# catid/siamese

Hardware: AMD Instinct MI355X
Metric: device-resident GB/s encode+decode, 1400B pkts @20% loss; % HBM peak (higher is better)
Workload: dtype u8

## Files before the change

siamese_amd/csrc/decoder.cpp:

```cpp
#include "decoder.h"

#include <algorithm>
#include <atomic>
#include <cstdio>
#include <cstdlib>
#include <cstring>
#include <x86intrin.h>

namespace sgpu {

namespace {

inline unsigned popcount_range(uint64_t bits, unsigned begin, unsigned end)
{
    if (begin >= end)
        return 0;
    uint64_t mask = (end >= 64 ? ~0ULL : ((1ULL << end) - 1)) & ~((1ULL << begin) - 1);
    return (unsigned)__builtin_popcountll(bits & mask);
}

inline unsigned first_clear(uint64_t bits, unsigned from)
{
    if (from >= 64)
        return 64;
    const uint64_t inv = ~bits & (~0ULL << from);
    return inv ? (unsigned)__builtin_ctzll(inv) : 64;
}

}

DecoderCore::DecoderCore(Engine* eng, bool hostMirror)
    : eng_(eng), prog_(eng, 1), mirror_(hostMirror)
{
    adopt_spare();
    if (!res_)
        res_ = std::make_shared<Resolver>();
    res_->mirror = mirror_;
}

struct DecoderCore::Spare
{
    std::vector<DecSubwindowPtr> subwindows;
    std::vector<SiameseOriginalPacket> recovered;
    std::vector<unsigned> recoveredColumns;
    std::vector<RowInfo> rows;
    std::vector<ColInfo> cols;
    std::vector<uint8_t> colLane, colCx, colCx2;
    std::vector<uint32_t> pickCol;
    std::vector<uint8_t> mat;
    std::vector<unsigned> pivots;
    std::shared_ptr<Resolver> res;
    std::vector<Fix> lastDecoded;
    std::vector<RecPacket*> scratchRec;
    std::vector<unsigned> scratchLen;
    std::vector<SolveRow> scratchRows;
    std::vector<uint8_t> scratchCoef;
    std::vector<unsigned> geEnd;
    std::vector<DevBuf> chainReleases;
    std::vector<unsigned> chainColumns;
    std::vector<uint32_t> geOut;
};

void DecoderCore::adopt_spare()
{
    Spare* s = CapStash<Spare>::take();
    if (!s)
        return;
    subwindows_.swap(s->subwindows);
    recovered_.swap(s->recovered);
    recoveredColumns_.swap(s->recoveredColumns);
    rows_.swap(s->rows);
    cols_.swap(s->cols);
    colLane_.swap(s->colLane);
    colCx_.swap(s->colCx);
    colCx2_.swap(s->colCx2);
    pickCol_.swap(s->pickCol);
    mat_.swap(s->mat);
    pivots_.swap(s->pivots);
    res_.swap(s->res);
    lastDecoded_.swap(s->lastDecoded);
    scratchRec_.swap(s->scratchRec);
    scratchLen_.swap(s->scratchLen);
    scratchRows_.swap(s->scratchRows);
    scratchCoef_.swap(s->scratchCoef);
    geEnd_.swap(s->geEnd);
    chainReleases_.swap(s->chainReleases);
    chainSums_.recoveredColumns.swap(s->chainColumns);
    geOut_.swap(s->geOut);
    CapStash<Spare>::put_shell(s);
}

void DecoderCore::donate_spare()
{
    Spare* s = CapStash<Spare>::shell();
    subwindows_.clear();
    recovered_.clear();
    recoveredColumns_.clear();
    rows_.clear();
    cols_.clear();
    colLane_.clear();
    colCx_.clear();
    colCx2_.clear();
    pickCol_.clear();
    pivots_.clear();
    if (res_ && res_.use_count() == 1) {
        for (PendingDecode& pd : res_->pend) {
            pd.fixes.clear();
            pd.words.clear();
            pd.targets.clear();
            pd.base = 0;
            pd.m = 0;
            pd.serial = 0;
            pd.live = false;
            pd.done = false;
            pd.held = false;
        }
        res_->doneCount.store(0, std::memory_order_relaxed);
        res_->orphan = false;
        res_->out = nullptr;
        res_->outCount = 0;
        res_->outSerial = 0;
        res_->geOut.clear();
        res_->geDone = false;
    } else if (res_) {
        std::lock_guard<std::mutex> g(res_->mu);
        res_->orphan = true;
        res_->out = nullptr;
        res_->outCount = 0;
        res_.reset();
    }
    lastDecoded_.clear();
    scratchRec_.clear();
    scratchLen_.clear();
    scratchRows_.clear();
    scratchCoef_.clear();
    geEnd_.clear();
    chainReleases_.clear();
    chainSums_.recoveredColumns.clear();
    geOut_.clear();
    subwindows_.swap(s->subwindows);
    recovered_.swap(s->recovered);
    recoveredColumns_.swap(s->recoveredColumns);
    rows_.swap(s->rows);
    cols_.swap(s->cols);
    colLane_.swap(s->colLane);
    colCx_.swap(s->colCx);
    colCx2_.swap(s->colCx2);
    pickCol_.swap(s->pickCol);
    mat_.swap(s->mat);
    pivots_.swap(s->pivots);
    res_.swap(s->res);
    lastDecoded_.swap(s->lastDecoded);
    scratchRec_.swap(s->scratchRec);
    scratchLen_.swap(s->scratchLen);
    scratchRows_.swap(s->scratchRows);
    scratchCoef_.swap(s->scratchCoef);
    geEnd_.swap(s->geEnd);
    chainReleases_.swap(s->chainReleases);
    chainSums_.recoveredColumns.swap(s->chainColumns);
    geOut_.swap(s->geOut);
    CapStash<Spare>::give(s);
}

DecoderCore::~DecoderCore()
{
    for (RecPacket* r = head_; r;) {
        RecPacket* n = r->next;
        free_packet(r);
        r = n;
    }
    for (auto& sw : subwindows_) {
        for (DecSlot& s : sw->slot) {
            if (!s.inSlab)
                eng_->release(s.buf);
            s.buf = DevBuf();
            s.inSlab = false;
            s.bytes = 0;
            s.column = 0;
            s.header = 0;
            s.pending = false;
            if (s.hostp)
                s.hostp->clear();
        }
        sw->got = 0;
        sw->gotCount = 0;
        eng_->slab_release(sw->slab);
        sw->slab = Slab();
        sw->clean = true;
    }
    for (auto& lane : lanes_)
        for (Sum& s : lane)
            eng_->release(s.d.buf);
    if (geState_ == 2)
        chain_sums_commit();
    donate_spare();
}


bool DecoderCore::mark_got(unsigned column)
{
    const unsigned element = column_to_element(column);
    if (element >= count_) {
        disabled_ = true;
        return false;
    }
    DecSubwindow* sw = subwindows_[element / kSubwindow].get();
    sw->gotCount++;
    sw->got |= 1ULL << (element % kSubwindow);
    return element == nextExpected_;
}

unsigned DecoderCore::range_lost(unsigned start, unsigned end)
{
    if (start >= end)
        return 0;
    unsigned lost = 0;
    unsigned sub = start / kSubwindow;
    const unsigned bitStart = start % kSubwindow;
    if (bitStart > 0) {
        unsigned bitEnd = bitStart + end - start;
        if (bitEnd > kSubwindow)
            bitEnd = kSubwindow;
        lost += (bitEnd - bitStart) - popcount_range(subwindows_[sub]->got, bitStart, bitEnd);
        ++sub;
    }
    const unsigned subEnd = end / kSubwindow;
    for (unsigned i = sub; i < subEnd; ++i)
        lost += kSubwindow - subwindows_[i]->gotCount;
    if (subEnd >= sub) {
        const unsigned lastBits = end - subEnd * kSubwindow;
        if (lastBits > 0)
            lost += lastBits - popcount_range(subwindows_[subEnd]->got, 0, lastBits);
    }
    return lost;
}

unsigned DecoderCore::find_next_lost(unsigned start)
{
    if (start >= count_)
        return count_;
    const unsigned subEnd = (count_ + kSubwindow - 1) / kSubwindow;
    unsigned sub = start / kSubwindow;
    unsigned bit = start % kSubwindow;
    while (sub < subEnd) {
        const DecSubwindow* sw = subwindows_[sub].get();
        if (sw->gotCount < kSubwindow) {
            bit = first_clear(sw->got, bit);
            if (bit < kSubwindow) {
                const unsigned e = sub * kSubwindow + bit;
                return e > count_ ? count_ : e;
            }
        }
        bit = 0;
        ++sub;
    }
    return count_;
}

void DecoderCore::iterate_next_expected(unsigned start)
{
    if (nextExpected_ >= count_)
        return;
    nextExpected_ = find_next_lost(start);
}

bool DecoderCore::grow_window(unsigned end)
{
    const unsigned needed = (end + kLanes + kSubwindow - 1) / kSubwindow;
    while (subwindows_.size() < needed) {
        subwindows_.emplace_back(ObjPool<DecSubwindow>::get());
        subwindows_.back()->clean = false;
    }
    if (end > count_)
        count_ = end;
    return true;
}

bool DecoderCore::place(unsigned element, unsigned need)
{
    DecSubwindow* sw = subwindows_[element / kSubwindow].get();
    DecSlot& s = sw->slot[element % kSubwindow];
    release_slot(s);
    bool failed = false;
    s.buf = eng_->slab_slot(sw->slab, element % kSubwindow, need, &failed);
    s.inSlab = (bool)s.buf;
    if (!s.buf && !failed)
        s.buf = eng_->alloc(need);
    return (bool)s.buf;
}

SiameseResult DecoderCore::accept_original(unsigned element, unsigned column, unsigned header, unsigned dataBytes)
{
    if (!place(element, header + dataBytes)) {
        disabled_ = true;
        return Siamese_Disabled;
    }
    DecSubwindow* sw = subwindows_[element / kSubwindow].get();
    const unsigned bit = element % kSubwindow;
    DecSlot& s = sw->slot[bit];
    s.header = header;
    s.bytes = header + dataBytes;
    s.column = column;
    s.pending = false;

    sw->gotCount++;
    sw->got |= 1ULL << bit;

    if (element == nextExpected_) {
        iterate_next_expected(element + 1);
        list_delete_before(nextExpected_);
    }
    if (element >= region_.elementStart && element < region_.nextCheckStart)
        region_reset();

    stats_[SiameseDecoderStats_OriginalCount]++;
    stats_[SiameseDecoderStats_OriginalBytes] += dataBytes;
    return Siamese_Success;
}

SiameseResult DecoderCore::add_original(const SiameseOriginalPacket& packet, uint64_t deviceSrc)
{
    settle();
    if (dead())
        return Siamese_Disabled;
    const unsigned element = column_to_element(packet.PacketNum);
    if (column_delta_negative(element)) {
        stats_[SiameseDecoderStats_DupedOriginalCount]++;
        return Siamese_DuplicateData;
    }
    grow_window(element + 1);
    DecSlot& s = slot(element);
    if (s.bytes > 0) {
        stats_[SiameseDecoderStats_DupedOriginalCount]++;
        return Siamese_DuplicateData;
    }

    uint8_t hdr[kMaxLengthPrefix];
    const unsigned h = write_length_prefix(packet.DataBytes, hdr);
    const SiameseResult r = accept_original(element, packet.PacketNum, h, packet.DataBytes);
    if (r != Siamese_Success)
        return r;
    if (deviceSrc)
        prog_.ingest_device(s.buf, deviceSrc, packet.DataBytes, hdr, h);
    else
        prog_.ingest_host(s.buf, packet.Data, packet.DataBytes, hdr, h);
    if (mirror_) {
        s.host().resize(h + packet.DataBytes);
        std::memcpy(s.host().data(), hdr, h);
        std::memcpy(s.host().data() + h, packet.Data, packet.DataBytes);
    }
    return Siamese_Success;
}

SiameseResult DecoderCore::add_original_range(unsigned firstNum, uint64_t src, uint32_t srcStride,
                                              const unsigned* lens, unsigned fixedBytes, unsigned count,
                                              SiameseResult* results, unsigned* added)
{
    *added = 0;
    settle();
    struct
    {
        uint64_t dst = 0, src = 0;
        uint32_t stride = 0, n = 0, bytes = 0, h = 0;
        uint8_t hdr[kMaxLengthPrefix] = {};
    } run;
    auto close_run = [&] {
        if (run.n)
            prog_.ingest_run(run.dst, run.stride, run.src, srcStride, run.n, run.bytes, run.hdr, run.h);
        run.n = 0;
    };
    SiameseResult res = Siamese_Success;
    for (unsigned k = 0; k < count; ++k) {
        const unsigned num = (firstNum + k) & SIAMESE_PACKET_NUM_MAX;
        const unsigned bytes = lens ? lens[k] : fixedBytes;
        SiameseResult r = Siamese_Success;
        const unsigned element = column_to_element(num);
        if (bytes == 0 || bytes > SIAMESE_MAX_PACKET_BYTES)
            r = Siamese_InvalidInput;
        else if (dead())
            r = Siamese_Disabled;
        else if (column_delta_negative(element))
            r = Siamese_DuplicateData;
        else {
            grow_window(element + 1);
            if (slot(element).bytes > 0)
                r = Siamese_DuplicateData;
        }
        if (r == Siamese_DuplicateData)
            stats_[SiameseDecoderStats_DupedOriginalCount]++;
        if (r == Siamese_Success) {
            uint8_t hdr[kMaxLengthPrefix];
            const unsigned h = write_length_prefix(bytes, hdr);
            r = accept_original(element, num, h, bytes);
            if (r == Siamese_Success) {
                const DecSlot& s = slot(element);
                const uint64_t from = src + (uint64_t)k * srcStride;
                if (run.n && run.bytes == bytes && run.n < kIngestRunMax && s.buf.cap == run.stride &&
                    s.buf.addr() == run.dst + (uint64_t)run.n * run.stride &&
                    from == run.src + (uint64_t)run.n * srcStride)
                    ++run.n;
                else {
                    close_run();
                    run.dst = s.buf.addr();
                    run.src = from;
                    run.stride = s.buf.cap;
                    run.n = 1;
                    run.bytes = bytes;
                    run.h = h;
                    std::memcpy(run.hdr, hdr, sizeof(hdr));
                }
            }
        }
        if (results)
            results[k] = r;
        ++*added;
        if (r != Siamese_Success && r != Siamese_DuplicateData) {
            res = r;
            break;
        }
    }
    close_run();
    return res;
}


bool DecoderCore::grow_sum(DevSum& s, unsigned bytes)
{
    if (bytes <= s.bytes)
        return true;
    if (bytes > s.buf.cap) {
        DevBuf nb = eng_->alloc(bytes);
        if (!nb) {
            disabled_ = true;
            return false;
        }
        if (s.devValid) {
            prog_.lc_begin(nb.addr(), s.devValid, 0);
            prog_.lc_term(s.buf.addr(), s.devValid, 1);
            prog_.lc_end();
        }
        release_sum_buf(s.buf);
        s.buf = nb;
    }
    s.bytes = bytes;
    return true;
}

void DecoderCore::cover(unsigned lo, unsigned hi)
{
    uint32_t from = hi;
    WinEntry* w = prog_.rows_window(lo, hi, &from);
    for (unsigned e = from; e < hi; ++e, ++w) {
        const DecSlot& o = slot(e);
        w->src = o.bytes ? o.buf.addr() : 0;
        w->len = o.bytes;
        w->column = o.bytes ? o.column : 0;
    }
}

void DecoderCore::materialize(unsigned lane, unsigned s)
{
    DevSum& d = sum(lane, s).d;
    if (d.devValid >= d.bytes)
        return;
    const unsigned at = sum(lane, s).elementEnd;
    const unsigned lo = std::min(at, windowLo_);
    cover(lo, lo);
    prog_.rows_update(lane * kSums + s, d.buf.addr(), d.bytes, d.devValid, s, at, at);
    d.devValid = d.bytes;
}

static uint8_t sum_coeff(unsigned sumIndex, unsigned column)
{
    if (sumIndex == 0)
        return 1;
    const uint8_t cx = column_value(column);
    return sumIndex == 2 ? gf_sqr(cx) : cx;
}

DevSum& DecoderCore::get_sum(unsigned lane, unsigned s, unsigned elementEnd)
{
    Sum& S = sum(lane, s);
    unsigned element = S.elementEnd;
    if (element >= elementEnd)
        return S.d;

    LaneScan& ls = laneScan_[lane];
    unsigned end = element;
    if (!(ls.from == element && ls.to == elementEnd && ls.epoch == scanEpoch_)) {
        unsigned most = 0, cnt = 0;
        for (; end < elementEnd; end += kLanes) {
            const unsigned b = slot(end).bytes;
            if (b > 0) {
                most = std::max(most, b);
                ++cnt;
            }
        }
        ls.from = element;
        ls.to = elementEnd;
        ls.end = end;
        ls.most = most;
        ls.got = cnt;
        ls.epoch = scanEpoch_;
    }
    end = ls.end;
    const unsigned got = ls.got;
    const unsigned newBytes = std::max(S.d.bytes, ls.most);
    if (got > 0) {
        if (!grow_sum(S.d, newBytes))
            return S.d;
        cover(std::min(element, windowLo_), end - kLanes + 1);
        prog_.rows_update(lane * kSums + s, S.d.buf.addr(), S.d.bytes, S.d.devValid, s, element, end);
        S.d.devValid = S.d.bytes;
    }
    S.elementEnd = end;
    return S.d;
}

bool DecoderCore::plug_sum_holes(unsigned elementStart)
{
    for (unsigned column : recoveredColumns_) {
        const unsigned element = column_to_element(column);
        if (element >= count_)
            continue;
        const unsigned lane = column % kLanes;
        const unsigned laneStart = next_lane_element(elementStart, lane);
        for (unsigned s = 0; s < kSums; ++s) {
            Sum& S = sum(lane, s);
            if (element < laneStart || element >= S.elementEnd)
                continue;
            const DecSlot& o = slot(element);
            if (o.bytes == 0)
                return false;
            if (!grow_sum(S.d, o.bytes))
                return false;
            prog_.lc_begin(S.d.buf.addr(), S.d.bytes, S.d.devValid);
            prog_.lc_term(o.buf.addr(), o.bytes, sum_coeff(s, column));
            prog_.lc_end();
            account_elim(o.bytes);
            S.d.devValid = S.d.bytes;
        }
    }
    recoveredColumns_.clear();
    return true;
}

void DecoderCore::reset_sums(unsigned elementStart)
{
    for (unsigned lane = 0; lane < kLanes; ++lane) {
        const unsigned laneStart = next_lane_element(elementStart, lane);
        for (unsigned s = 0; s < kSums; ++s) {
            Sum& S = sum(lane, s);
            S.elementStart = laneStart;
            S.elementEnd = laneStart;
            S.d.bytes = 0;
            S.d.devValid = 0;
        }
    }
    recoveredColumns_.clear();
}

bool DecoderCore::start_sums(unsigned elementStart, unsigned bufferBytes)
{
    for (unsigned lane = 0; lane < kLanes; ++lane) {
        const unsigned laneStart = next_lane_element(elementStart, lane);
        for (unsigned s = 0; s < kSums; ++s) {
            Sum& S = sum(lane, s);
            if (S.d.bytes == 0) {
                S.elementEnd = laneStart;
            } else if (S.elementStart != laneStart) {
                S.elementEnd = laneStart;
                S.d.bytes = 0;
                S.d.devValid = 0;
            }
            S.elementStart = laneStart;
            if (!grow_sum(S.d, bufferBytes))
                return false;
        }
    }
    if (!recoveredColumns_.empty() && !plug_sum_holes(elementStart))
        return false;
    return true;
}


void DecoderCore::remove_elements()
{
    if (nextExpected_ < kRemoveThreshold)
        return;

    unsigned firstKept = 0;
    unsigned targetStart = 0, targetCount = 0, initialBytes = 0;
    bool seenSum = false;

    const RecPacket* r = head_;
    if (!r) {
        const RowMeta m = lastMeta_;
        const unsigned end = column_to_element(m.columnStart + m.sumCount);
        if (column_delta_negative(end) || end < m.ldpcCount) {
            disabled_ = true;
            return;
        }
        firstKept = end - m.ldpcCount;
        targetStart = m.columnStart;
        targetCount = m.sumCount;
        initialBytes = lastBytes_;
        if (m.sumCount > kCauchyThreshold)
            seenSum = true;
    } else {
        firstKept = r->elementStart;
        initialBytes = r->bytes;
        for (;;) {
            const unsigned sc = r->meta.sumCount;
            const unsigned cs = r->meta.columnStart;
            if (sc > kCauchyThreshold) {
                if (!seenSum) {
                    targetStart = cs;
                    targetCount = sc;
                    seenSum = true;
                } else if (cs != targetStart || sc < targetCount) {
                    const unsigned firstSum = column_to_element(cs);
                    if (firstSum >= count_) {
                        disabled_ = true;
                        return;
                    }
                    if (firstKept > firstSum)
                        firstKept = firstSum;
                }
            }
            r = r->next;
            if (!r)
                break;
            if (firstKept > r->elementStart)
                firstKept = r->elementStart;
            if (initialBytes < r->bytes)
                initialBytes = r->bytes;
        }
    }

    if (firstKept < kRemoveThreshold)
        return;

    const unsigned keptSub = firstKept / kSubwindow;
    const unsigned removed = keptSub * kSubwindow;

    if (seenSum) {
        unsigned sumElementStart = column_to_element(targetStart);
        if (sumColumnStart_ != targetStart || sumColumnCount_ > targetCount) {
            if (sumElementStart >= count_) {
                disabled_ = true;
                return;
            }
            reset_sums(sumElementStart);
            sumColumnStart_ = targetStart;
            sumColumnCount_ = targetCount;
        } else {
            if (sumElementStart >= count_)
                sumElementStart = 0;
            if (!start_sums(sumElementStart, initialBytes)) {
                disabled_ = true;
                return;
            }
        }
        ++scanEpoch_;
        for (unsigned lane = 0; lane < kLanes; ++lane) {
            for (unsigned s = 0; s < kSums; ++s) {
                get_sum(lane, s, removed);
                Sum& S = sum(lane, s);
                if (S.elementStart >= removed)
                    S.elementStart -= removed;
                else
                    S.elementStart = lane;
                S.elementEnd -= removed;
            }
        }
    } else {
        sumColumnCount_ = 0;
    }

    prog_.rows_seal();
    for (unsigned i = 0; i < keptSub; ++i) {
        DecSubwindow* sw = subwindows_[i].get();
        for (DecSlot& d : sw->slot)
            if (d.inSlab) {
                d.buf = DevBuf();
                d.inSlab = false;
            }
        eng_->slab_release(sw->slab);
        sw->reset();
    }
    std::rotate(subwindows_.begin(), subwindows_.begin() + keptSub, subwindows_.end());

    count_ -= removed;
    columnStart_ = element_to_column(removed);
    nextExpected_ -= removed;

    for (RecPacket* p = head_; p; p = p->next) {
        p->elementEnd -= removed;
        p->elementStart -= removed;
    }
    if (region_.elementStart < removed || region_.nextCheckStart < removed)
        region_reset();
    else {
        region_.elementStart -= removed;
        region_.nextCheckStart -= removed;
    }
    prevNextCheckStart_ = prevNextCheckStart_ > removed ? prevNextCheckStart_ - removed : 0;
}


void DecSubwindowRecycle::operator()(DecSubwindow* w) const
{
    if (!w->clean) {
        w->got = 0;
        w->gotCount = 0;
        w->slab = Slab();
        for (DecSlot& s : w->slot) {
            s.buf = DevBuf();
            s.inSlab = false;
            s.bytes = 0;
            s.column = 0;
            s.header = 0;
            s.pending = false;
            if (s.hostp)
                s.hostp->clear();
        }
        w->clean = true;
    }
    ObjPool<DecSubwindow>::put(w);
}

void DecoderCore::free_packet(RecPacket* r)
{
    eng_->release(r->buf);
    *r = RecPacket();
    ObjPool<RecPacket>::put(r);
}

void DecoderCore::list_insert(RecPacket* r, bool outOfOrder)
{
    RecPacket* prev = tail_;
    RecPacket* next = nullptr;
    const unsigned rs = r->meta.columnStart;
    const unsigned re = r->elementEnd;
    for (; prev; next = prev, prev = prev->prev) {
        const unsigned pe = prev->elementEnd;
        if (re >= pe) {
            if (re > pe)
                break;
            if (column_delta_negative(column_sub(rs, prev->meta.columnStart)))
                break;
        }
    }
    r->next = next;
    r->prev = prev;
    if (prev)
        prev->next = r;
    else
        head_ = r;
    if (next)
        next->prev = r;
    else
        tail_ = r;
    if (!prev || next)
        region_reset();
    ++listCount_;
    if (!outOfOrder) {
        lastMeta_ = r->meta;
        lastBytes_ = r->bytes;
    }
}

void DecoderCore::list_delete_before(unsigned element)
{
    RecPacket* r = head_;
    unsigned deleted = 0;
    bool regionStale = false;
    while (r && r->elementEnd <= element) {
        RecPacket* n = r->next;
        if (r == region_.first || r == region_.last)
            regionStale = true;
        free_packet(r);
        ++deleted;
        r = n;
    }
    if (regionStale)
        region_reset();
    head_ = r;
    if (r) {
        r->prev = nullptr;
        listCount_ -= deleted;
    } else {
        tail_ = nullptr;
        listCount_ = 0;
    }
}


SiameseResult DecoderCore::add_recovery(const SiameseRecoveryPacket& packet)
{
    settle();
    if (dead())
        return Siamese_Disabled;
    RowMeta m;
    const int footer = read_footer(packet.Data, packet.DataBytes, &m);
    if (footer < 0) {
        disabled_ = true;
        return Siamese_Disabled;
    }
    return add_recovery_common(m, footer, packet.DataBytes, packet.Data, 0, packet.Data, nullptr);
}

SiameseResult DecoderCore::add_recovery_device(const DeviceRecovery& rec)
{
    settle();
    if (dead())
        return Siamese_Disabled;
    RowMeta m;
    int footer = read_footer(rec.footer, rec.footerBytes, &m);
    if (footer < 0 || (unsigned)footer != rec.footerBytes) {
        disabled_ = true;
        return Siamese_Disabled;
    }
    return add_recovery_common(m, footer, rec.bytes, nullptr, rec.data, rec.head, rec.producer);
}

SiameseResult DecoderCore::add_recovery_common(const RowMeta& m, int footer, unsigned totalBytes,
                                               const void* hostData, uint64_t devData,
                                               const uint8_t* headBytes, Program* producer)
{
    stats_[SiameseDecoderStats_RecoveryCount]++;
    stats_[SiameseDecoderStats_RecoveryBytes] += totalBytes;

    const bool outOfOrder = column_delta_negative(m.columnStart + m.sumCount - latestColumn_);
    if (!outOfOrder)
        latestColumn_ = (m.columnStart + m.sumCount) % kColumnPeriod;

    unsigned elementStart, elementEnd;
    if (count_ == 0) {
        if (outOfOrder) {
            stats_[SiameseDecoderStats_DupedRecoveryCount]++;
            return Siamese_Success;
        }
        columnStart_ = m.columnStart;
        grow_window(m.sumCount);
        elementEnd = m.sumCount;
        elementStart = elementEnd - m.ldpcCount;
    } else {
        elementEnd = column_to_element(m.columnStart + m.sumCount);
        if (column_delta_negative(elementEnd) || elementEnd < m.ldpcCount) {
            stats_[SiameseDecoderStats_DupedRecoveryCount]++;
            return Siamese_Success;
        }
        elementStart = elementEnd - m.ldpcCount;
        if (elementEnd <= nextExpected_) {
            if (outOfOrder) {
                stats_[SiameseDecoderStats_DupedRecoveryCount]++;
                return Siamese_Success;
            }
            if (elementStart >= kRemoveThreshold) {
                lastMeta_ = m;
                lastBytes_ = totalBytes - footer;
                remove_elements();
            }
            stats_[SiameseDecoderStats_DupedRecoveryCount]++;
            return Siamese_Success;
        }
        if (m.sumCount > kCauchyThreshold) {
            if (sumColumnCount_ == 0 || sumColumnStart_ != m.columnStart) {
                if (column_to_element(m.columnStart) >= count_) {
                    stats_[SiameseDecoderStats_DupedRecoveryCount]++;
                    return Siamese_Success;
                }
            }
        }
        grow_window(elementEnd);
    }

    const unsigned payload = totalBytes - footer;
    if (m.sumCount == 1) {
        if (!add_single(m, headBytes, payload, hostData, devData, producer)) {
            disabled_ = true;
            return Siamese_Disabled;
        }
        return Siamese_Success;
    }

    RecPacket* r = ObjPool<RecPacket>::get();
    r->buf = eng_->alloc(payload + payload / 16);
    if (!r->buf) {
        ObjPool<RecPacket>::put(r);
        disabled_ = true;
        return Siamese_Disabled;
    }
    static const uint8_t none[1] = {0};
    if (hostData)
        prog_.ingest_host(r->buf, hostData, payload, none, 0);
    else if (!producer)
        prog_.ingest_device(r->buf, devData, payload, none, 0);
    else {
        (void)producer;
        prog_.copy(r->buf.addr(), devData, payload);
    }
    r->bytes = payload;
    r->meta = m;
    r->elementStart = elementStart;
    r->elementEnd = elementEnd;
    list_insert(r, outOfOrder);
    if (elementStart >= kRemoveThreshold)
        remove_elements();
    return Siamese_Success;
}

bool DecoderCore::add_single(const RowMeta& m, const uint8_t* headBytes, unsigned payloadBytes,
                             const void* hostData, uint64_t devData, Program* producer)
{
    const unsigned element = column_to_element(m.columnStart);
    if (element >= count_)
        return false;
    DecSlot& s = slot(element);
    if (s.bytes != 0)
        return true;

    unsigned length = 0;
    const int headerBytes = read_length_prefix(headBytes, std::min(payloadBytes, kMaxLengthPrefix), &length);
    if (headerBytes < 1 || length == 0 || length + (unsigned)headerBytes != payloadBytes)
        return false;

    uint8_t hdr[kMaxLengthPrefix];
    const unsigned h = write_length_prefix(length, hdr);
    if (!place(element, h + length))
        return false;
    if (hostData)
        prog_.ingest_host(s.buf, (const uint8_t*)hostData + headerBytes, length, hdr, h);
    else if ((unsigned)headerBytes == h && producer) {
        prog_.copy(s.buf.addr(), devData, h + length);
    } else
        prog_.ingest_device(s.buf, devData + headerBytes, length, hdr, h);
    if (mirror_) {
        s.host().resize(h + length);
        std::memcpy(s.host().data(), hdr, h);
        std::memcpy(s.host().data() + h, (const uint8_t*)hostData + headerBytes, length);
    }
    s.header = h;
    s.bytes = h + length;
    s.column = m.columnStart;
    s.pending = false;

    {
        std::lock_guard<std::mutex> g(res_->mu);
        if (!hasRecovered_) {
            hasRecovered_ = true;
            recovered_.clear();
            ++decodeSerial_;
        }
        SiameseOriginalPacket out;
        out.PacketNum = m.columnStart;
        out.DataBytes = length;
        out.Data = (mirror_ ? s.host().data() : s.buf.ptr) + h;
        recovered_.push_back(out);
        publish_outputs();
    }
    recoveredColumns_.push_back(m.columnStart);

    if (element >= region_.elementStart && element < region_.nextCheckStart)
        region_reset();

    if (mark_got(m.columnStart)) {
        iterate_next_expected(element + 1);
        list_delete_before(nextExpected_);
        if (region_.nextCheckStart >= kRemoveThreshold)
            remove_elements();
    }
    return true;
}


void DecoderCore::matrix_reset()
{
    cols_.clear();
    rows_.clear();
    pivots_.clear();
    matRows_ = matCols_ = 0;
    prevNextCheckStart_ = 0;
    geResume_ = 0;
}

void DecoderCore::region_reset()
{
    region_.elementStart = 0;
    region_.nextCheckStart = 0;
    region_.first = nullptr;
    region_.last = nullptr;
    region_.recoveryCount = 0;
    region_.lostCount = 0;
    region_.solveFailed = false;
    matrix_reset();
}

bool DecoderCore::check_recovery_possible()
{
    if (dead())
        return false;
    RecPacket* r;
    unsigned nextCheck, recCount, lost;
    if (!region_.last) {
        r = head_;
        if (!r)
            return false;
        region_.first = r;
        region_.elementStart = r->elementStart;
        recCount = 1;
        nextCheck = r->elementEnd;
        lost = range_lost(r->elementStart, nextCheck);
        region_.solveFailed = false;
        r->lostCount = lost;
    } else {
        recCount = region_.recoveryCount;
        lost = region_.lostCount;
        if (recCount >= lost && !region_.solveFailed)
            return lost <= kMaxLossRecovery;
        r = region_.last;
        nextCheck = region_.nextCheckStart;
    }
    while ((recCount < lost || region_.solveFailed) && r->next) {
        r = r->next;
        ++recCount;
        unsigned end = r->elementEnd;
        if (end < nextCheck)
            end = nextCheck;
        lost += range_lost(nextCheck, end);
        nextCheck = end;
        r->lostCount = lost;
        region_.solveFailed = false;
    }
    region_.last = r;
    region_.recoveryCount = recCount;
    region_.lostCount = lost;
    region_.nextCheckStart = nextCheck;
    if (lost > kMaxLossRecovery)
        return false;
    return recCount >= lost && !region_.solveFailed;
}

SiameseResult DecoderCore::is_ready()
{
    settle();
    if (hasRecovered_ || check_recovery_possible())
        return Siamese_Success;
    return Siamese_NeedMoreData;
}

SiameseResult DecoderCore::decode(SiameseOriginalPacket** packetsOut, unsigned* countOut)
{
    settle();
    if (dead())
        return Siamese_Disabled;
    if (hasRecovered_) {
        hasRecovered_ = false;
        if (packetsOut) {
            *packetsOut = recovered_.data();
            *countOut = (unsigned)recovered_.size();
        }
        return Siamese_Success;
    }
    if (packetsOut) {
        *packetsOut = nullptr;
        *countOut = 0;
    }
    if (!check_recovery_possible())
        return Siamese_NeedMoreData;
    return decode_loop(packetsOut, countOut);
}

SiameseResult DecoderCore::decode_loop(SiameseOriginalPacket** packetsOut, unsigned* countOut)
{
    RecPacket* r = region_.last;
    unsigned nextCheck = region_.nextCheckStart;
    unsigned recCount = region_.recoveryCount;
    unsigned lost = region_.lostCount;

    for (;;) {
        if (recCount >= lost) {
            const SiameseResult res = decode_region();
            if (res == Siamese_Success) {
                if (packetsOut) {
                    *packetsOut = recovered_.data();
                    *countOut = (unsigned)recovered_.size();
                }
                return Siamese_Success;
            }
            if (res != Siamese_NeedMoreData)
                return res;
        }
        if (!r->next)
            break;
        r = r->next;
        ++recCount;
        unsigned end = r->elementEnd;
        if (end < nextCheck)
            end = nextCheck;
        lost += range_lost(nextCheck, end);
        r->lostCount = lost;
        nextCheck = end;
    }
    region_.last = r;
    region_.nextCheckStart = nextCheck;
    region_.recoveryCount = recCount;
    region_.lostCount = lost;
    return Siamese_NeedMoreData;
}

namespace {
const bool kDecodeClocks = std::getenv("SIAMESE_AMD_DECODE_CLOCKS") != nullptr;
struct DecodeClocks
{
    std::atomic<uint64_t> n{0}, rows{0}, cols{0}, fails{0}, fresh{0}, t[4];
    std::mutex mu;
    std::vector<uint32_t> samples[4];
    void sample(const uint64_t* d)
    {
        std::lock_guard<std::mutex> g(mu);
        for (int k = 0; k < 4; ++k)
            if (samples[k].size() < (1u << 16))
                samples[k].push_back((uint32_t)d[k]);
    }
    ~DecodeClocks()
    {
        if (!kDecodeClocks || !n)
            return;
        double med[4] = {0, 0, 0, 0};
        for (int k = 0; k < 4; ++k)
            if (!samples[k].empty()) {
                std::nth_element(samples[k].begin(), samples[k].begin() + samples[k].size() / 2, samples[k].end());
                med[k] = samples[k][samples[k].size() / 2];
            }
        std::fprintf(stderr, "decode_region medians (ticks): generate %.0f ge %.0f eliminate %.0f solve %.0f\n",
                     med[0], med[1], med[2], med[3]);
        std::fprintf(stderr, "decode_region %llu solved, %llu failed, %llu fresh matrices, rows %.1f cols %.1f; "
                     "ticks/solved call: generate %.0f ge %.0f eliminate %.0f solve %.0f\n",
                     (unsigned long long)n.load(), (unsigned long long)fails.load(), (unsigned long long)fresh.load(),
                     (double)rows / (n + fails), (double)cols / (n + fails), (double)t[0] / n, (double)t[1] / n,
                     (double)t[2] / n, (double)t[3] / n);
    }
} g_decodeClocks;
struct ChainClocks
{
    std::mutex mu;
    std::vector<uint32_t> samples[4];
    void sample(const uint64_t* d)
    {
        std::lock_guard<std::mutex> g(mu);
        for (int k = 0; k < 4; ++k)
            if (samples[k].size() < (1u << 16))
                samples[k].push_back((uint32_t)d[k]);
    }
    ~ChainClocks()
    {
        if (!kDecodeClocks || samples[0].empty())
            return;
        double med[4] = {0, 0, 0, 0};
        for (int k = 0; k < 4; ++k)
            if (!samples[k].empty()) {
                std::nth_element(samples[k].begin(), samples[k].begin() + samples[k].size() / 2, samples[k].end());
                med[k] = samples[k][samples[k].size() / 2];
            }
        std::fprintf(stderr, "chained decode medians (ticks): job %.0f eliminate %.0f solve %.0f finish %.0f\n",
                     med[0], med[1], med[2], med[3]);
    }
} g_chainClocks;
thread_local uint64_t t_chain[3];
}

SiameseResult DecoderCore::decode_region()
{
    uint64_t c0 = kDecodeClocks ? __rdtsc() : 0, c1 = 0, c2 = 0, c3 = 0;
    const size_t oldRowsAtEntry = rows_.size();
    geBytes_ = 0;
    if (!generate_matrix()) {
        disabled_ = true;
        return Siamese_Disabled;
    }
    if (kDecodeClocks)
        c1 = __rdtsc();
    const bool solved = gaussian_elimination();
    eng_->account(geBytes_);
    if (kDecodeClocks) {
        c2 = __rdtsc();
        g_decodeClocks.rows += matRows_;
        g_decodeClocks.cols += matCols_;
        g_decodeClocks.fails += solved ? 0 : 1;
        g_decodeClocks.fresh += oldRowsAtEntry == 0 ? 1 : 0;
    }
    if (!solved)
        return finish_region(false);
    if (!eliminate_original_data()) {
        disabled_ = true;
        return Siamese_Disabled;
    }
    if (kDecodeClocks)
        c3 = __rdtsc();
    const SiameseResult res = solve_and_substitute();
    if (kDecodeClocks) {
        const uint64_t c4 = __rdtsc();
        g_decodeClocks.n++;
        g_decodeClocks.t[0] += c1 - c0;
        g_decodeClocks.t[1] += c2 - c1;
        g_decodeClocks.t[2] += c3 - c2;
        g_decodeClocks.t[3] += c4 - c3;
        const uint64_t d[4] = {c1 - c0, c2 - c1, c3 - c2, c4 - c3};
        g_decodeClocks.sample(d);
    }
    region_reset();
    return res;
}

SiameseResult DecoderCore::finish_region(bool solved)
{
    if (!solved) {
        region_.solveFailed = true;
        stats_[SiameseDecoderStats_SolveFailCount]++;
        return Siamese_NeedMoreData;
    }
    if (!eliminate_original_data()) {
        disabled_ = true;
        return Siamese_Disabled;
    }
    const SiameseResult res = solve_and_substitute();
    region_reset();
    return res;
}


SiameseResult DecoderCore::decode_device(SiameseOriginalPacket** packetsOut, unsigned* countOut)
{
    if (geState_)
        return finish_device_ge(packetsOut, countOut);
    settle();
    if (dead())
        return Siamese_Disabled;
    if (hasRecovered_) {
        hasRecovered_ = false;
        if (packetsOut) {
            *packetsOut = recovered_.data();
            *countOut = (unsigned)recovered_.size();
        }
        return Siamese_Success;
    }
    if (packetsOut) {
        *packetsOut = nullptr;
        *countOut = 0;
    }
    if (!check_recovery_possible())
        return Siamese_NeedMoreData;
    if (region_.recoveryCount >= region_.lostCount && rows_.empty() && geResume_ == 0 && !geHost_ &&
        (submit_chained() || submit_device_ge()))
        return kDecodePending;
    return decode_loop(packetsOut, countOut);
}

bool DecoderCore::submit_device_ge(bool chained)
{
    const unsigned columns = region_.lostCount;
    const unsigned rows = region_.recoveryCount;
    if (columns == 0 || columns > kGeMaxCols || rows > kGeMaxRows)
        return false;
    matrix_resize(rows, columns, true);
    populate_columns(0, columns);
    populate_rows(0, rows);
    unsigned pickLo = ~0u, pickHi = 0;
    for (unsigned i = 0; i < rows; ++i) {
        const RecPacket* rec = rows_[i].rec;
        if (rec->meta.sumCount <= kCauchyThreshold)
            continue;
        pickLo = std::min(pickLo, rec->elementStart);
        pickHi = std::max(pickHi, rec->elementStart + rec->meta.ldpcCount);
    }
    const unsigned pickLen = pickHi > pickLo ? pickHi - pickLo : 0;
    if (disabled_ || pickLen > kGeMaxPick) {
        disabled_ = false;
        matrix_reset();
        return false;
    }
    uint32_t base = 0;
    uint8_t* in = prog_.ge_job(rows, columns, pickLen, &base, chained);
    GeRow* R = reinterpret_cast<GeRow*>(in);
    GeCol* C = reinterpret_cast<GeCol*>(R + rows);
    uint8_t* pick = reinterpret_cast<uint8_t*>(C + columns);
    for (unsigned j = 0; j < columns; ++j)
        C[j] = GeCol{colLane_[j], colCx_[j], colCx2_[j], (uint8_t)(cols_[j].column % kCauchyMaxColumns)};
    for (unsigned e = pickLo; e < pickHi; ++e) {
        const DecSlot& a = slot(e);
        pick[e - pickLo] = (a.bytes == 0 && a.column < columns) ? (uint8_t)a.column : kGeNoColumn;
    }
    unsigned endKeyStart = ~0u, endKeyCount = 0, endVal = 0;
    for (unsigned i = 0; i < rows; ++i) {
        const RecPacket* rec = rows_[i].rec;
        const RowMeta m = rec->meta;
        unsigned jEnd = 0;
        if (endKeyStart == m.columnStart && endKeyCount == m.sumCount)
            jEnd = endVal;
        else {
            while (jEnd < columns && column_sub(cols_[jEnd].column, m.columnStart) < m.sumCount)
                ++jEnd;
            endKeyStart = m.columnStart;
            endKeyCount = m.sumCount;
            endVal = jEnd;
        }
        GeRow& g = R[i];
        std::memset(&g, 0, sizeof(g));
        g.jEnd = (uint16_t)jEnd;
        g.colCount = (uint16_t)rows_[i].columnCount;
        if (m.sumCount <= kCauchyThreshold) {
            g.kind = m.row == 0 ? GE_PARITY : GE_CAUCHY;
            g.rbase = (uint8_t)(m.row - 1 + kCauchyMaxColumns);
        } else {
            g.kind = GE_SIAMESE;
            g.row = (uint16_t)m.row;
            g.ldpcN = m.ldpcCount;
            g.pickOff = rec->elementStart - pickLo;
        }
    }
    const uint32_t words = ge_result_words(rows, columns, chained);
    prog_.on_complete(res_, [r = res_.get(), base, words](const uint32_t* results) {
        std::lock_guard<std::mutex> g(r->mu);
        r->geOut.assign(results + base, results + base + words);
        r->geDone = true;
    });
    geState_ = chained ? 2 : 1;
    EngineStats& st = eng_->shard().stats;
    st.geJobs++;
    st.geChained += chained ? 1 : 0;
    geRows_ = rows;
    geCols_ = columns;
    geBase_ = base;
    return true;
}

bool DecoderCore::submit_chained()
{
    const unsigned columns = region_.lostCount;
    const unsigned rows = region_.recoveryCount;
    if (mirror_ || rows != columns || columns == 0 || columns > kGeMaxCols)
        return false;
    const uint64_t c0 = kDecodeClocks ? __rdtsc() : 0;
    const RecPacket* r = region_.first;
    const unsigned bytes = r->bytes;
    for (unsigned i = 0; i < rows; ++i, r = r->next)
        if (r->bytes != bytes)
            return false;
    if (!submit_device_ge(true))
        return false;
    const uint64_t c1 = kDecodeClocks ? __rdtsc() : 0;
    pivots_.resize(rows);
    for (unsigned i = 0; i < rows; ++i) {
        rows_[i].used = true;
        pivots_[i] = i;
    }
    const uint32_t okWord = geBase_ + 3;
    for (unsigned l = 0; l < kLanes; ++l)
        for (unsigned k = 0; k < kSums; ++k)
            chainSums_.lanes[l][k] = lanes_[l][k];
    chainSums_.columnStart = sumColumnStart_;
    chainSums_.columnCount = sumColumnCount_;
    chainSums_.recoveredColumns = recoveredColumns_;
    chainReleases_.clear();
    prog_.gate_begin(okWord);
    deferAccount_ = true;
    deferRelease_ = true;
    deferredBytes_ = 0;
    chainElimFailed_ = !eliminate_original_data();
    deferAccount_ = false;
    deferRelease_ = false;
    if (prog_.gate_end())
        eng_->shard().stats.geChainedWide++;
    const uint64_t c2 = kDecodeClocks ? __rdtsc() : 0;
    chainSlot_ = ~0u;
    chainBytes_ = bytes;
    if (!chainElimFailed_) {
        unsigned slot = 0;
        if (solve_plan(okWord + 1, &slot))
            chainSlot_ = slot;
        else
            chainElimFailed_ = true;
    }
    if (kDecodeClocks) {
        t_chain[0] = c1 - c0;
        t_chain[1] = c2 - c1;
        t_chain[2] = __rdtsc() - c2;
    }
    return true;
}

SiameseResult DecoderCore::finish_chained(SiameseOriginalPacket** packetsOut, unsigned* countOut)
{
    const unsigned columns = geCols_;
    const uint32_t* o = geOut_.data();
    const bool ok = o[3] != 0;
#ifdef SGPU_GE_CLOCKS
    static struct GeClocks
    {
        std::atomic<uint64_t> n{0}, t[3];
        std::mutex mu;
        std::vector<std::pair<uint32_t, uint32_t>> jobs;
        ~GeClocks()
        {
// ... 1027 lines not shown
```

siamese_amd/csrc/decoder.h:

```cpp
#pragma once

#include "codedef.h"
#include "encoder.h"
#include "engine.h"
#include "gf.h"
#include "objpool.h"
#include "../../include/siamese.h"

#include <atomic>
#include <memory>
#include <mutex>
#include <vector>

namespace sgpu {

constexpr SiameseResult kDecodePending = static_cast<SiameseResult>(6);
constexpr SiameseResult kNeedsFlush = static_cast<SiameseResult>(7);

struct DecSlot
{
    DevBuf buf;
    bool inSlab = false;
    unsigned bytes = 0;
    unsigned column = 0;
    unsigned header = 0;
    bool pending = false;
    uint32_t pendSlot = 0;
    uint32_t pendCi = 0;
    std::unique_ptr<std::vector<uint8_t>> hostp;
    std::vector<uint8_t>& host()
    {
        if (!hostp)
            hostp.reset(new std::vector<uint8_t>);
        return *hostp;
    }
};

struct DecSubwindow
{
    DecSlot slot[kSubwindow];
    uint64_t got = 0;
    unsigned gotCount = 0;
    Slab slab;
    bool clean = false;
    void reset()
    {
        got = 0;
        gotCount = 0;
        for (DecSlot& s : slot) {
            s.column = 0;
            s.bytes = 0;
            s.pending = false;
        }
    }
};

struct DecSubwindowRecycle
{
    void operator()(DecSubwindow* w) const;
};
using DecSubwindowPtr = std::unique_ptr<DecSubwindow, DecSubwindowRecycle>;

struct RecPacket
{
    RecPacket* next = nullptr;
    RecPacket* prev = nullptr;
    RowMeta meta;
    unsigned elementStart = 0;
    unsigned elementEnd = 0;
    unsigned lostCount = 0;
    DevBuf buf;
    unsigned bytes = 0;
};

struct DeviceRecovery
{
    uint64_t data = 0;
    unsigned bytes = 0;
    const uint8_t* footer = nullptr;
    unsigned footerBytes = 0;
    const uint8_t* head = nullptr;
    Program* producer = nullptr;
};

class DecoderCore
{
public:
    DecoderCore(Engine* eng, bool hostMirror);
    ~DecoderCore();

    Program& program() { return prog_; }

    SiameseResult add_original(const SiameseOriginalPacket& packet, uint64_t deviceSrc = 0);
    SiameseResult add_original_range(unsigned firstNum, uint64_t src, uint32_t srcStride, const unsigned* lens,
                                     unsigned fixedBytes, unsigned count, SiameseResult* results,
                                     unsigned* added);
    SiameseResult get_range(unsigned firstNum, unsigned count, SiameseOriginalPacket* out, unsigned* got);
    SiameseResult add_recovery(const SiameseRecoveryPacket& packet);
    SiameseResult add_recovery_device(const DeviceRecovery& rec);
    SiameseResult is_ready();
    SiameseResult decode(SiameseOriginalPacket** packetsOut, unsigned* countOut);
    SiameseResult decode_device(SiameseOriginalPacket** packetsOut, unsigned* countOut);
    bool ge_pending() const { return geState_ != 0; }
    SiameseResult get(SiameseOriginalPacket& packet);
    SiameseResult decode_deferred(SiameseOriginalPacket* out, unsigned capacity, unsigned* countOut);
    SiameseResult get_deferred(SiameseOriginalPacket& packet);
    void settle()
    {
        if (res_->doneCount.load(std::memory_order_acquire) != appliedCount_)
            apply_resolved();
    }
    SiameseResult stats(uint64_t* out, unsigned count);
    SiameseResult acknowledgement(uint8_t* buffer, unsigned byteLimit, unsigned& usedBytes);

    bool disabled()
    {
        settle();
        return dead();
    }
    bool dead() const { return disabled_ || eng_->failed(); }
    bool has(unsigned packetNum)
    {
        settle();
        const unsigned e = column_to_element(packetNum);
        return !dead() && e < count_ && slot(e).bytes > 0;
    }
    bool pending(unsigned packetNum)
    {
        settle();
        const unsigned e = column_to_element(packetNum);
        return !dead() && e < count_ && slot(e).bytes > 0 && slot(e).pending;
    }
    bool has_pending() const { return pendingSolves_ > 0; }
    void download_recovered();

private:
    DecSlot& slot(unsigned e) { return subwindows_[e / kSubwindow]->slot[e % kSubwindow]; }
    unsigned column_to_element(unsigned c) const { return column_sub(c, columnStart_); }
    unsigned element_to_column(unsigned e) const { return column_add(e, columnStart_); }
    unsigned next_lane_element(unsigned element, unsigned lane) const
    {
        unsigned e = element - (element % kLanes) + lane;
        return e < element ? e + kLanes : e;
    }
    bool mark_got(unsigned column);
    bool place(unsigned element, unsigned need);
    void release_slot(DecSlot& s)
    {
        if (!s.inSlab)
            eng_->release(s.buf);
        s.buf = DevBuf();
        s.inSlab = false;
    }
    SiameseResult accept_original(unsigned element, unsigned column, unsigned header, unsigned dataBytes);
    unsigned range_lost(unsigned start, unsigned end);
    unsigned find_next_lost(unsigned start);
    unsigned find_next_got(unsigned start);
    void iterate_next_expected(unsigned start);
    bool grow_window(unsigned end);

    struct Sum
    {
        unsigned elementStart = 0, elementEnd = 0;
        DevSum d;
    };
    Sum& sum(unsigned lane, unsigned s) { return lanes_[lane][s]; }
    bool grow_sum(DevSum& s, unsigned bytes);
    void materialize(unsigned lane, unsigned s);
    void cover(unsigned lo, unsigned hi);
    unsigned windowLo_ = 0;
    DevSum& get_sum(unsigned lane, unsigned s, unsigned elementEnd);
    struct LaneScan
    {
        unsigned from = ~0u, to = 0, end = 0, most = 0, got = 0;
        uint64_t epoch = ~0ull;
    };
    LaneScan laneScan_[kLanes];
    uint64_t scanEpoch_ = 0;
    bool start_sums(unsigned elementStart, unsigned bufferBytes);
    void reset_sums(unsigned elementStart);
    bool plug_sum_holes(unsigned elementStart);
    void remove_elements();

    void list_insert(RecPacket* r, bool outOfOrder);
    void list_delete_before(unsigned element);
    void free_packet(RecPacket* r);

    void region_reset();
    void matrix_reset();
    bool check_recovery_possible();
    SiameseResult decode_region();
    SiameseResult decode_loop(SiameseOriginalPacket** packetsOut, unsigned* countOut);
    SiameseResult finish_region(bool solved);
    bool submit_device_ge(bool chained = false);
    SiameseResult finish_device_ge(SiameseOriginalPacket** packetsOut, unsigned* countOut);
    bool submit_chained();
    SiameseResult finish_chained(SiameseOriginalPacket** packetsOut, unsigned* countOut);
    unsigned geState_ = 0;
    unsigned geRows_ = 0, geCols_ = 0;
    uint32_t geBase_ = 0;
    std::vector<uint32_t> geOut_;
    bool deferAccount_ = false;
    uint64_t deferredBytes_ = 0;
    bool chainElimFailed_ = false;
    unsigned chainSlot_ = 0;
    unsigned chainBytes_ = 0;
    void account_elim(uint64_t bytes)
    {
        if (deferAccount_)
            deferredBytes_ += bytes;
        else
            eng_->account(bytes);
    }
    struct SumState
    {
        Sum lanes[kLanes][kSums];
        unsigned columnStart = 0, columnCount = 0;
        std::vector<unsigned> recoveredColumns;
    };
    SumState chainSums_;
    bool deferRelease_ = false;
    std::vector<DevBuf> chainReleases_;
    void release_sum_buf(DevBuf& b)
    {
        if (deferRelease_) {
            chainReleases_.push_back(b);
            b = DevBuf();
        } else {
            eng_->release(b);
        }
    }
    void chain_sums_commit();
    void chain_sums_restore();
    bool generate_matrix();
    void populate_columns(unsigned oldColumns, unsigned newColumns);
    void populate_rows(unsigned oldRows, unsigned newRows);
    void resume_ge(unsigned oldRows, unsigned rows);
    bool gaussian_elimination();
    bool pivoted_ge(unsigned pivot);
    bool eliminate_row(const uint8_t* geRow, uint8_t* remRow, unsigned pivot, unsigned end,
                       uint8_t valI);
    uint8_t* mrow(unsigned r) { return mat_.data() + (size_t)r * matStride_; }
    bool matrix_resize(unsigned rows, unsigned columns, bool initialize);

    bool eliminate_original_data();
    SiameseResult solve_and_substitute();
    bool solve_plan(uint32_t gateWord, unsigned* slotOut);
    SiameseResult solve_publish(unsigned slot);
    SiameseResult publish_final(unsigned slot);

    bool add_single(const RowMeta& m, const uint8_t* headBytes, unsigned payloadBytes,
                    const void* hostData, uint64_t devData, Program* producer);
    SiameseResult add_recovery_common(const RowMeta& m, int footerBytes, unsigned totalBytes,
                                      const void* hostData, uint64_t devData,
                                      const uint8_t* headBytes, Program* producer);

    Engine* eng_;
    Program prog_;
    bool mirror_;
    bool disabled_ = false;

    unsigned count_ = 0;
    unsigned columnStart_ = 0;
    unsigned nextExpected_ = 0;
    std::vector<DecSubwindowPtr> subwindows_;
    Sum lanes_[kLanes][kSums];
    unsigned sumColumnStart_ = 0;
    unsigned sumColumnCount_ = 0;
    std::vector<SiameseOriginalPacket> recovered_;
    bool hasRecovered_ = false;
    std::vector<unsigned> recoveredColumns_;

    RecPacket* head_ = nullptr;
    RecPacket* tail_ = nullptr;
    unsigned listCount_ = 0;
    RowMeta lastMeta_;
    unsigned lastBytes_ = 0;

    struct
    {
        unsigned elementStart = 0;
        RecPacket* first = nullptr;
        RecPacket* last = nullptr;
        unsigned nextCheckStart = 0;
        unsigned recoveryCount = 0, lostCount = 0;
        bool solveFailed = false;
    } region_;

    struct RowInfo
    {
        RecPacket* rec = nullptr;
        bool used = false;
        unsigned columnCount = 0;
    };
    struct ColInfo
    {
        DecSlot* original = nullptr;
        unsigned column = 0;
    };
    std::vector<RowInfo> rows_;
    std::vector<ColInfo> cols_;
    static constexpr unsigned kRowSlack = 32;
    std::vector<uint8_t> colLane_, colCx_, colCx2_;
    std::vector<uint32_t> pickCol_;
    unsigned prevNextCheckStart_ = 0;
    std::vector<uint8_t> mat_;
    unsigned matRows_ = 0, matCols_ = 0, matAllocRows_ = 0, matStride_ = 0;
    std::vector<unsigned> pivots_;
    std::vector<unsigned> geEnd_;
    unsigned geResume_ = 0;
    bool geHost_ = false;
    uint64_t geBytes_ = 0;
    GfRowSrc geSrc_;
    const uint8_t* geSrcRow_ = nullptr;
    unsigned geSrcPivot_ = 0;

    unsigned latestColumn_ = 0;

    struct Fix
    {
        DecSlot* slot;
        uint8_t* buf;
        uint32_t resultWord;
        unsigned outIndex;
        unsigned bound;
    };
    struct PendingDecode
    {
        std::vector<Fix> fixes;
        uint32_t base = 0;
        unsigned m = 0;
        uint64_t serial = 0;
        bool live = false;
        bool done = false;
        bool held = false;
        std::vector<uint32_t> words;
        std::vector<std::pair<unsigned, SiameseOriginalPacket*>> targets;
    };
    struct Resolver
    {
        std::mutex mu;
        std::vector<PendingDecode> pend;
        std::atomic<uint64_t> doneCount{0};
        bool orphan = false;
        SiameseOriginalPacket* out = nullptr;
        size_t outCount = 0;
        uint64_t outSerial = 0;
        bool mirror = false;
        std::vector<uint32_t> geOut;
        bool geDone = false;
    };
    static void complete_solve(Resolver& r, unsigned slot, const uint32_t* results);
    static void fill_entry(const PendingDecode& pd, unsigned ci, SiameseOriginalPacket& out);
    void apply_resolved();
    void publish_outputs();
    std::shared_ptr<Resolver> res_;
    uint64_t appliedCount_ = 0;
    unsigned lastPendSlot_ = 0;
    std::vector<Fix> lastDecoded_;
    std::vector<RecPacket*> scratchRec_;
    std::vector<unsigned> scratchLen_;
    std::vector<SolveRow> scratchRows_;
    std::vector<uint8_t> scratchCoef_;
    uint64_t decodeSerial_ = 0;

    struct Spare;
    void adopt_spare();
    void donate_spare();
    unsigned pendingSolves_ = 0;

    uint64_t stats_[SiameseDecoderStats_Count] = {};
};

}
```

Before: 3503.

## Memoize recovery-region walk and shortcut same-key list inserts in decoder

Adds generation counters for the loss window and the recovery packet list, and caches the result of the from-head recovery walk so that a later check after a single head insertion can reuse it instead of re-walking the list. It also remembers the first packet of the tail run sharing the same key, so inserts that match the tail skip the backward linear scan. These target host-side O(n) list traversals in the decoder's bookkeeping. The cost is extra state that must be invalidated correctly everywhere the window or list changes, with debug-only checkers to verify equivalence.

```diff
diff --git a/siamese_amd/csrc/decoder.cpp b/siamese_amd/csrc/decoder.cpp
--- a/siamese_amd/csrc/decoder.cpp
+++ b/siamese_amd/csrc/decoder.cpp
@@ -27,11 +27,35 @@
     return inv ? (unsigned)__builtin_ctzll(inv) : 64;
 }
 
+#if defined(SGPU_WALK_CHECK) && !defined(SGPU_WALK_COUNT)
+#define SGPU_WALK_COUNT
+#endif
+#ifdef SGPU_WALK_COUNT
+struct WalkCounts
+{
+    std::atomic<uint64_t> decoders{0}, inserts{0}, insertHops{0}, checks{0}, checkVisits{0}, shortcuts{0};
+    ~WalkCounts()
+    {
+        if (!std::getenv("SIAMESE_AMD_WALK_COUNTS"))
+            return;
+        std::fprintf(stderr, "walk counts: decoders %llu inserts %llu insert_hops %llu checks %llu "
+                     "check_visits %llu shortcuts %llu\n",
+                     (unsigned long long)decoders.load(), (unsigned long long)inserts.load(),
+                     (unsigned long long)insertHops.load(), (unsigned long long)checks.load(),
+                     (unsigned long long)checkVisits.load(), (unsigned long long)shortcuts.load());
+    }
+} g_walk;
+#define SGPU_WALK_VISIT(field) ((void)g_walk.field.fetch_add(1, std::memory_order_relaxed))
+#else
+#define SGPU_WALK_VISIT(field) ((void)0)
+#endif
+
 }
 
 DecoderCore::DecoderCore(Engine* eng, bool hostMirror)
     : eng_(eng), prog_(eng, 1), mirror_(hostMirror)
 {
+    SGPU_WALK_VISIT(decoders);
     adopt_spare();
     if (!res_)
         res_ = std::make_shared<Resolver>();
@@ -169,6 +193,8 @@
         free_packet(r);
         r = n;
     }
+    head_ = tail_ = runFirst_ = nullptr;
+    walkMemo_.valid = false;
     for (auto& sw : subwindows_) {
         for (DecSlot& s : sw->slot) {
             if (!s.inSlab)
@@ -207,6 +233,7 @@
     DecSubwindow* sw = subwindows_[element / kSubwindow].get();
     sw->gotCount++;
     sw->got |= 1ULL << (element % kSubwindow);
+    ++windowGen_;
     return element == nextExpected_;
 }
 
@@ -262,6 +289,7 @@
     if (nextExpected_ >= count_)
         return;
     nextExpected_ = find_next_lost(start);
+    ++windowGen_;
 }
 
 bool DecoderCore::grow_window(unsigned end)
@@ -270,9 +298,12 @@
     while (subwindows_.size() < needed) {
         subwindows_.emplace_back(ObjPool<DecSubwindow>::get());
         subwindows_.back()->clean = false;
-    }
-    if (end > count_)
+        ++windowGen_;
+    }
+    if (end > count_) {
         count_ = end;
+        ++windowGen_;
+    }
     return true;
 }
 
@@ -305,6 +336,7 @@
 
     sw->gotCount++;
     sw->got |= 1ULL << bit;
+    ++windowGen_;
 
     if (element == nextExpected_) {
         iterate_next_expected(element + 1);
@@ -694,6 +726,7 @@
     count_ -= removed;
     columnStart_ = element_to_column(removed);
     nextExpected_ -= removed;
+    ++windowGen_;
 
     for (RecPacket* p = head_; p; p = p->next) {
         p->elementEnd -= removed;
@@ -743,7 +776,25 @@
     RecPacket* next = nullptr;
     const unsigned rs = r->meta.columnStart;
     const unsigned re = r->elementEnd;
+#ifndef SGPU_WALK_FULL
+    const bool tailKey = tail_ && re == tail_->elementEnd && rs == tail_->meta.columnStart;
+#else
+    const bool tailKey = false;
+#endif
+    if (tailKey) {
+        if (!runFirst_) {
+            runFirst_ = tail_;
+            while (runFirst_->prev && runFirst_->prev->elementEnd == re &&
+                   runFirst_->prev->meta.columnStart == rs) {
+                runFirst_ = runFirst_->prev;
+                SGPU_WALK_VISIT(insertHops);
+            }
+        }
+        next = runFirst_;
+        prev = runFirst_->prev;
+    }
     for (; prev; next = prev, prev = prev->prev) {
+        SGPU_WALK_VISIT(insertHops);
         const unsigned pe = prev->elementEnd;
         if (re >= pe) {
             if (re > pe)
@@ -752,6 +803,20 @@
                 break;
         }
     }
+    SGPU_WALK_VISIT(inserts);
+#ifdef SGPU_WALK_CHECK
+    {
+        RecPacket* p = tail_;
+        RecPacket* n = nullptr;
+        for (; p; n = p, p = p->prev) {
+            const unsigned pe = p->elementEnd;
+            if (re > pe || (re == pe && column_delta_negative(column_sub(rs, p->meta.columnStart))))
+                break;
+        }
+        if (p != prev || n != next)
+            walk_check_failed("list_insert: position differs from the search from the tail");
+    }
+#endif
     r->next = next;
     r->prev = prev;
     if (prev)
@@ -762,6 +827,11 @@
         next->prev = r;
     else
         tail_ = r;
+    if (!next)
+        runFirst_ = r;
+    else if (tailKey && next == runFirst_)
+        runFirst_ = r;
+    ++listGen_;
     if (!prev || next)
         region_reset();
     ++listCount_;
@@ -780,10 +850,14 @@
         RecPacket* n = r->next;
         if (r == region_.first || r == region_.last)
             regionStale = true;
+        if (r == runFirst_)
+            runFirst_ = nullptr;
         free_packet(r);
         ++deleted;
         r = n;
     }
+    if (deleted)
+        ++listGen_;
     if (regionStale)
         region_reset();
     head_ = r;
@@ -843,6 +917,7 @@
             return Siamese_Success;
         }
         columnStart_ = m.columnStart;
+        ++windowGen_;
         grow_window(m.sumCount);
         elementEnd = m.sumCount;
         elementStart = elementEnd - m.ldpcCount;
@@ -1004,10 +1079,21 @@
         return false;
     RecPacket* r;
     unsigned nextCheck, recCount, lost;
-    if (!region_.last) {
+    SGPU_WALK_VISIT(checks);
+    const bool fromHead = !region_.last;
+    if (fromHead) {
         r = head_;
         if (!r)
             return false;
+        if (walk_shortcut()) {
+#ifdef SGPU_WALK_CHECK
+            walk_check();
+#endif
+            if (region_.lostCount > kMaxLossRecovery)
+                return false;
+            return region_.recoveryCount >= region_.lostCount;
+        }
+        SGPU_WALK_VISIT(checkVisits);
         region_.first = r;
         region_.elementStart = r->elementStart;
         recCount = 1;
@@ -1023,7 +1109,10 @@
         r = region_.last;
         nextCheck = region_.nextCheckStart;
     }
+    bool walked = fromHead;
     while ((recCount < lost || region_.solveFailed) && r->next) {
+        SGPU_WALK_VISIT(checkVisits);
+        walked = true;
         r = r->next;
         ++recCount;
         unsigned end = r->elementEnd;
@@ -1038,10 +1127,82 @@
     region_.recoveryCount = recCount;
     region_.lostCount = lost;
     region_.nextCheckStart = nextCheck;
+    if (walked) {
+        walkMemo_.valid = fromHead && !r->next && recCount < lost && head_->lostCount == lost;
+        if (walkMemo_.valid) {
+            walkMemo_.head = head_;
+            walkMemo_.tail = r;
+            walkMemo_.elementStart = head_->elementStart;
+            walkMemo_.elementEnd = head_->elementEnd;
+            walkMemo_.windowGen = windowGen_;
+            walkMemo_.listGen = listGen_;
+            walkMemo_.listCount = listCount_;
+            walkMemo_.lost = lost;
+            walkMemo_.nextCheckStart = nextCheck;
+            walkMemo_.recoveryCount = recCount;
+        }
+    }
     if (lost > kMaxLossRecovery)
         return false;
     return recCount >= lost && !region_.solveFailed;
 }
+
+bool DecoderCore::walk_shortcut()
+{
+    const RecPacket* h = head_;
+#ifdef SGPU_WALK_FULL
+    walkMemo_.valid = false;
+#endif
+    if (!walkMemo_.valid || windowGen_ != walkMemo_.windowGen || listGen_ != walkMemo_.listGen + 1 ||
+        h->next != walkMemo_.head || tail_ != walkMemo_.tail || listCount_ != walkMemo_.listCount + 1 ||
+        h->elementStart != walkMemo_.elementStart || h->elementEnd != walkMemo_.elementEnd)
+        return false;
+    head_->lostCount = walkMemo_.lost;
+    region_.first = head_;
+    region_.elementStart = head_->elementStart;
+    region_.last = tail_;
+    region_.recoveryCount = walkMemo_.recoveryCount + 1;
+    region_.lostCount = walkMemo_.lost;
+    region_.nextCheckStart = walkMemo_.nextCheckStart;
+    region_.solveFailed = false;
+    walkMemo_.valid = region_.recoveryCount < region_.lostCount;
+    walkMemo_.head = head_;
+    walkMemo_.listGen = listGen_;
+    walkMemo_.listCount = listCount_;
+    walkMemo_.recoveryCount = region_.recoveryCount;
+    SGPU_WALK_VISIT(shortcuts);
+    return true;
+}
+
+#ifdef SGPU_WALK_CHECK
+void DecoderCore::walk_check_failed(const char* what)
+{
+    std::fprintf(stderr, "SGPU_WALK_CHECK: %s\n", what);
+    std::abort();
+}
+
+void DecoderCore::walk_check()
+{
+    RecPacket* r = head_;
+    unsigned recCount = 1, nextCheck = r->elementEnd;
+    unsigned lost = range_lost(r->elementStart, nextCheck);
+    bool same = r->lostCount == lost;
+    while (recCount < lost && r->next) {
+        r = r->next;
+        ++recCount;
+        unsigned end = r->elementEnd;
+        if (end < nextCheck)
+            end = nextCheck;
+        lost += range_lost(nextCheck, end);
+        nextCheck = end;
+        same = same && r->lostCount == lost;
+    }
+    if (!same || region_.first != head_ || region_.elementStart != head_->elementStart || region_.last != r ||
+        region_.recoveryCount != recCount || region_.lostCount != lost || region_.nextCheckStart != nextCheck ||
+        region_.solveFailed)
+        walk_check_failed("check_recovery_possible: the shortcut differs from the walk");
+}
+#endif
 
 SiameseResult DecoderCore::is_ready()
 {
@@ -1102,6 +1263,7 @@
             end = nextCheck;
         lost += range_lost(nextCheck, end);
         r->lostCount = lost;
+        walkMemo_.valid = false;
         nextCheck = end;
     }
     region_.last = r;
diff --git a/siamese_amd/csrc/decoder.h b/siamese_amd/csrc/decoder.h
--- a/siamese_amd/csrc/decoder.h
+++ b/siamese_amd/csrc/decoder.h
@@ -276,6 +276,9 @@
     unsigned listCount_ = 0;
     RowMeta lastMeta_;
     unsigned lastBytes_ = 0;
+    RecPacket* runFirst_ = nullptr;
+    uint64_t listGen_ = 0;
+    uint64_t windowGen_ = 0;
 
     struct
     {
@@ -286,6 +289,21 @@
         unsigned recoveryCount = 0, lostCount = 0;
         bool solveFailed = false;
     } region_;
+    struct
+    {
+        bool valid = false;
+        RecPacket* head = nullptr;
+        RecPacket* tail = nullptr;
+        unsigned elementStart = 0, elementEnd = 0;
+        uint64_t windowGen = 0, listGen = 0;
+        unsigned listCount = 0;
+        unsigned lost = 0, nextCheckStart = 0, recoveryCount = 0;
+    } walkMemo_;
+    bool walk_shortcut();
+#ifdef SGPU_WALK_CHECK
+    void walk_check();
+    [[noreturn]] static void walk_check_failed(const char* what);
+#endif
 
     struct RowInfo
     {
```

Result: faster. 3662, median of 6 (+4.5%).
